# edsonportosilva/OptiCommPy

Hardware: AMD Instinct MI355X
Metric: SSFM steps/sec (2-pol, 2^20 samples) (higher is better)
Workload: dtype f64

## Files before the change

opticommpy_amd/csrc/engine_fused_impl.h:

```cpp
#pragma once
#include <algorithm>
#include <cstdlib>
#include <vector>

#include "dev_ctx.h"
#include "fused_engine.h"
#include "ssf_internal.h"

namespace ssf {
namespace {

using namespace fused;

#ifdef SSF_PHASE_TIMING
__device__ unsigned long long g_marks[4][4096][8];
#endif

struct DevCtx : DevCtxCore {
#ifdef SSF_PHASE_TIMING
    int kind;
    unsigned long long ts[8] = {0, 0, 0, 0, 0, 0, 0, 0};
    __device__ __forceinline__ void mark(int i) {
        __builtin_amdgcn_sched_barrier(0);
#if SSF_PHASE_TIMING != 2
// ... 689 lines not shown
        if (std::memcmp(k5, key, sizeof(key)) != 0) {
            const double w2 = (w_scale / (double)N) * (w_scale / (double)N);
            LinOp lo = make_linop(hzh, lin_a, lin_b, w2, scale, 4);
            be.h2d(lin_d, &lo, sizeof(LinOp));
            std::memcpy(key, k5, sizeof(key));
        }
        RowArgs<T> a{};
        a.G = (cx<T> *)out;
        a.src = in == out ? nullptr : (const cx<T> *)in;
        a.log2N1 = 0;
        a.log2N2 = 0;
        a.nfft = nrows;
        a.use_ctrl = 0;
        a.lin = lin_d;
        a.N2 = (int)N;
        a.N = N;
        a.mixed = 1;
        a.plan = plan;
        a.wtab = use_wtab ? wtab : nullptr;
        a.rows_per_wg = rows_wg;
        be.launch_row(a, nrows / rows_wg, tpr * rows_wg, 4096 + (size_t)rows_wg * (size_t)N * sizeof(cx<T>));
        return be.ok() ? SSF_OK : SSF_ERR_HIP;
    }
};

template <typename T>
int overlap_save_t(int64_t sigLen, int nrows, int lg, int K, const void *Hfft, const void *in, void *out, std::string *err) {
    using Cc = cx<T>;
    const int nfft = 1 << lg, d = nfft - K + 1, discard = K - 1, D = (K - 1) / 2;
    const long long numBlocks = (sigLen + K - 1 + d - 1) / d;
    const size_t sig_bytes = sizeof(Cc) * (size_t)sigLen * (size_t)nrows;
    hipStream_t st = nullptr;
    Cc *din = nullptr, *dout = nullptr, *dH = nullptr;
    auto fail_ = [&](const char *what, hipError_t e) {
        *err = std::string(what) + ": " + hipGetErrorString(e);
        if (din) (void)hipFree(din);
        if (dout) (void)hipFree(dout);
        if (dH) (void)hipFree(dH);
        if (st) (void)hipStreamDestroy(st);
        return e == hipErrorOutOfMemory ? SSF_ERR_OOM : SSF_ERR_HIP;
    };
    hipError_t e;
    if ((e = hipStreamCreateWithFlags(&st, hipStreamNonBlocking)) != hipSuccess) return fail_("hipStreamCreate", e);
    if ((e = hipMalloc(&din, sig_bytes)) != hipSuccess) return fail_("hipMalloc", e);
    if ((e = hipMalloc(&dout, sig_bytes)) != hipSuccess) return fail_("hipMalloc", e);
    if ((e = hipMalloc(&dH, sizeof(Cc) * (size_t)nfft)) != hipSuccess) return fail_("hipMalloc", e);
    std::vector<Cc> Hs((size_t)nfft);
    for (int i = 0; i < nfft; ++i) {
        Hs[(size_t)i].re = ((const Cc *)Hfft)[i].re / (T)nfft;
        Hs[(size_t)i].im = ((const Cc *)Hfft)[i].im / (T)nfft;
    }
    ols_permute_filter(Hs.data(), lg);
    Stager stg;
    (void)stg.init();
    if ((e = stg.h2d(din, in, sig_bytes, st)) != hipSuccess) return fail_("upload", e);
    if ((e = hipMemcpyAsync(dH, Hs.data(), sizeof(Cc) * (size_t)nfft, hipMemcpyHostToDevice, st)) != hipSuccess) return fail_("upload H", e);
    OlsArgs<T> a{};
    a.in = din;
    a.out = dout;
    a.H = dH;
    a.sigLen = sigLen;
    a.njobs = numBlocks * nrows;
    a.nrows = nrows;
    a.log2nfft = lg;
    a.d = d;
    a.discard = discard;
    a.D = D;
    ols_defaults(a);
    const int tpf = nfft / 16;
    const int block = tpf >= 256 ? tpf : 256, fpw = block / tpf;
    const long long grid = (a.njobs + fpw - 1) / fpw;
    const size_t lds = (size_t)fpw * lds_slots_per_fft(nfft) * sizeof(Cc);
    if (block <= 256) {
        (void)hipFuncSetAttribute((const void *)k_ols<T, 256>, hipFuncAttributeMaxDynamicSharedMemorySize, 160 * 1024);
        k_ols<T, 256><<<(unsigned)grid, block, lds, st>>>(a);
    } else {
        (void)hipFuncSetAttribute((const void *)k_ols<T, 1024>, hipFuncAttributeMaxDynamicSharedMemorySize, 160 * 1024);
        k_ols<T, 1024><<<(unsigned)grid, block, lds, st>>>(a);
    }
    if ((e = hipGetLastError()) != hipSuccess) return fail_("launch k_ols", e);
    if ((e = stg.d2h(out, dout, sig_bytes, st)) != hipSuccess) return fail_("download", e);
    (void)hipFree(din);
    (void)hipFree(dout);
    (void)hipFree(dH);
    (void)hipStreamDestroy(st);
    return SSF_OK;
}

inline int couple_reduce_selftest_impl(int nranks, int npart, const double *parts, double *out5, std::string *err) {
    if (nranks < 1 || npart < 1 || !parts || !out5) return SSF_ERR_BAD_ARG;
    double *d = nullptr, *work = nullptr;
    const size_t n = (size_t)nranks * 5 * (size_t)npart;
    hipError_t e = hipMalloc(&d, sizeof(double) * n);
    if (e == hipSuccess) e = hipMalloc(&work, sizeof(double) * (size_t)(8 + 5 * nranks));
    if (e == hipSuccess) e = hipMemcpy(d, parts, sizeof(double) * n, hipMemcpyHostToDevice);
    for (int r = 0; r < nranks && e == hipSuccess; ++r) {
        const double *b = d + (size_t)r * 5 * npart;
        CoupleArgs a{b + 3 * (size_t)npart, b + 4 * (size_t)npart, b + (size_t)npart, b + 2 * (size_t)npart, b, npart, work + 8 + 5 * r};
        k_couple_local<<<1, 256>>>(a);
        e = hipGetLastError();
    }
    if (e == hipSuccess) {
        k_couple_finish<<<1, 64>>>(work + 8, nranks, work);
        e = hipGetLastError();
    }
    if (e == hipSuccess) e = hipMemcpy(out5, work, sizeof(double) * 5, hipMemcpyDeviceToHost);
    if (d) (void)hipFree(d);
// ... 38 lines not shown
```

opticommpy_amd/csrc/engine_rx.hip:

```cpp
#include <cstring>
#include <set>
#include <string>
#include <utility>
#include <vector>

#include "dev_ctx.h"
#include "rx_pipeline.h"
#include "ssf_copy.h"
#include "ssf_internal.h"

namespace ssf {
namespace {

using namespace rx;

struct RxCtx : DevCtxCore {
    __device__ __forceinline__ void mark(int) {}
    __device__ __forceinline__ void flush(int) {}
};
#define SSF_RX_CTX()                                                          \
    extern __shared__ __attribute__((aligned(16))) char ssf_smem[];           \
    RxCtx ctx{{(int)threadIdx.x, (int)blockIdx.x, (int)blockDim.x, (int)gridDim.x, ssf_smem}}

template <int LG, int C> __global__ void __launch_bounds__(fused::ols_threads(LG, C)) k_rx_ols(const fused::OlsArgs<double> a) {
// ... 37 lines not shown
    absmax_body(ctx, a);
}
__global__ void __launch_bounds__(256) k_tx_phase_noise(const PnArgs a) {
    SSF_RX_CTX();
    pn_body(ctx, a);
}
__global__ void __launch_bounds__(256) k_tx_iqm(const IqmArgs a) {
    SSF_RX_CTX();
    iqm_body(ctx, a);
}
__global__ void __launch_bounds__(256) k_tx_shift_add(const ShiftAddArgs a) {
    SSF_RX_CTX();
    shift_add_body(ctx, a);
}
template <int LG, int C, int MODE> __global__ void __launch_bounds__(fused::ols_threads(LG, C)) k_rx_chain_ols(const ChainOlsArgs a) {
    SSF_RX_CTX();
    chain_ols_body<LG, C, MODE>(ctx, a);
}
__global__ void __launch_bounds__(1024) k_rx_chain_finish(const ChainFinishArgs a) {
    SSF_RX_CTX();
    chain_finish_body(ctx, a);
}
__global__ void __launch_bounds__(256) k_rx_dec_stats(const DecStatsArgs a) {
    SSF_RX_CTX();
    dec_stats_body(ctx, a);
}
__global__ void __launch_bounds__(256) k_rx_dec_sum(const DecSumArgs a) {
    SSF_RX_CTX();
    dec_sum_body(ctx, a);
}
__global__ void __launch_bounds__(256) k_rx_dec_finish(const DecFinishArgs a) {
    SSF_RX_CTX();
    dec_finish_body(ctx, a);
}
__global__ void __launch_bounds__(256) k_rx_dec_gather(const DecGatherArgs a) {
    SSF_RX_CTX();
    dec_gather_body(ctx, a);
}

struct HipRxBackend {
    hipStream_t st = nullptr;
    hipError_t first_err = hipSuccess;
    std::string where;
    Stager stg;
    void chk(hipError_t e, const char *what) {
        if (e != hipSuccess && first_err == hipSuccess) {
            first_err = e;
            where = what;
        }
    }
    int open(int device) {
        chk(hipSetDevice(device), "hipSetDevice");
        chk(hipStreamCreateWithFlags(&st, hipStreamNonBlocking), "hipStreamCreate");
        if (ok()) chk(stg.init(), "pinned staging buffers");
        return ok() ? SSF_OK : SSF_ERR_HIP;
    }
    ~HipRxBackend() {
        if (st) (void)hipStreamDestroy(st);
    }
    bool ok() const { return first_err == hipSuccess; }
    bool oom() const { return first_err == hipErrorOutOfMemory; }
    std::string last_error() const { return where + ": " + hipGetErrorString(first_err); }
    void *alloc(size_t n) {
        void *p = nullptr;
        hipError_t e = hipMalloc(&p, n);
        if (e != hipSuccess) {
            chk(e, "hipMalloc");
            return nullptr;
        }
        return p;
    }
    void free(void *p) { (void)hipFree(p); }
    void h2d(void *d, const void *h, size_t n) {
        chk(hipMemcpyAsync(d, h, n, hipMemcpyHostToDevice, st), "hipMemcpyAsync H2D");
        chk(hipStreamSynchronize(st), "hipStreamSynchronize");
    }
    void d2h(void *h, const void *d, size_t n) {
        chk(hipMemcpyAsync(h, d, n, hipMemcpyDeviceToHost, st), "hipMemcpyAsync D2H");
        chk(hipStreamSynchronize(st), "hipStreamSynchronize");
    }
    void h2d_big(void *d, const void *h, size_t n) { chk(stg.h2d(d, h, n, st), "staged upload"); }
    void d2h_big(void *h, const void *d, size_t n) { chk(stg.d2h(h, d, n, st), "staged download"); }
    void sync() { chk(hipStreamSynchronize(st), "hipStreamSynchronize"); }
    static unsigned ew_grid(long long n) {
        const long long g = (n + 255) / 256;
        return (unsigned)(g < 1 ? 1 : g > 4096 ? 4096 : g);
    }
    std::set<const void *> armed;
    template <class K> void arm(K kernel) {
        if (!armed.insert((const void *)kernel).second) return;
        chk(hipFuncSetAttribute((const void *)kernel, hipFuncAttributeMaxDynamicSharedMemorySize, 160 * 1024), "hipFuncSetAttribute");
    }
    void launch_ols(const fused::OlsArgs<double> &a) {
        const fused::OlsLaunch o = fused::ols_launch(a.log2nfft, a.nrows, a.njobs);
        fused::ols_dispatch(o, [&](auto lg, auto cc) {
            constexpr int LG = decltype(lg)::value, C = decltype(cc)::value;
            arm(k_rx_ols<LG, C>);
            k_rx_ols<LG, C><<<(unsigned)o.grid, o.threads, o.lds_bytes, st>>>(a);
        });
        chk(hipGetLastError(), "launch k_rx_ols");
    }
    void launch_rx_ols(const RxOlsArgs &a) {
        const fused::OlsLaunch o = fused::ols_launch(a.o.log2nfft, a.o.nrows, a.o.njobs);
        const bool found = rx_ols_dispatch(a, o, [&](auto lg, auto cc, auto pre, auto noise) {
            constexpr int LG = decltype(lg)::value, C = decltype(cc)::value, PRE = decltype(pre)::value, NOISE = decltype(noise)::value;
            arm(k_rx_ols_fused<LG, C, PRE, NOISE>);
            k_rx_ols_fused<LG, C, PRE, NOISE><<<(unsigned)o.grid, o.threads, o.lds_bytes, st>>>(a);
// ... 246 lines not shown
```

opticommpy_amd/csrc/ssf_api.hip:

```cpp
#include <map>
#include <memory>
#include <thread>

#include "ssf_internal.h"

using namespace ssf;

namespace {
thread_local std::string g_err;

int set_err(int code, const std::string &m) {
    g_err = m;
    return code;
}

int check_params(ssf_plan *pl, const ssf_params *p, int s0, int s1) {
    if (!p) return fail(pl, SSF_ERR_BAD_ARG, "params is NULL");
    if (p->model != SSF_MODEL_NLSE && p->model != SSF_MODEL_MANAKOV) return fail(pl, SSF_ERR_BAD_ARG, "bad model");
    if (p->model == SSF_MODEL_MANAKOV && (pl->nrows % 2)) return fail(pl, SSF_ERR_BAD_ARG, "Manakov model needs an even number of rows");
    if (p->model == SSF_MODEL_NLSE && p->direction < 0) return fail(pl, SSF_ERR_BAD_ARG, "NLSE model has no back-propagation mode");
    if (!(p->Fs > 0) || !(p->Fc > 0)) return fail(pl, SSF_ERR_BAD_ARG, "Fs and Fc must be positive");
    if (!(p->Lspan > 0)) return fail(pl, SSF_ERR_BAD_ARG, "Lspan must be positive");
    if (!(p->hz > 0) && !(p->model == SSF_MODEL_MANAKOV && p->nlprMethod)) return fail(pl, SSF_ERR_BAD_ARG, "hz must be positive");
    if (p->model == SSF_MODEL_MANAKOV && p->maxIter < 1) return fail(pl, SSF_ERR_BAD_ARG, "maxIter must be >= 1");
// ... 177 lines not shown
                ssf_stats *stats, ssf_trace *trace) {
    if (!plan) return set_err(SSF_ERR_BAD_ARG, "plan is NULL");
    if (!plan->has_field) return fail(plan, SSF_ERR_STATE, "ssf_execute before ssf_upload");
    int rc = check_params(plan, params, span_first, span_last);
    if (!rc && plan->sink.active()) {
        long long ncap = 0;
        for (int i = 0; i < params->n_save; ++i)
            if (params->save_spans[i] >= span_first && params->save_spans[i] <= span_last) ++ncap;
        if (((long long)plan->sink.count() + ncap) * plan->nrows > plan->sink.leading())
            return fail(plan, SSF_ERR_BAD_ARG, "snapshot sink: the captures of this call do not fit the destination's columns");
    }
    if (rc) return rc;
    SSF_HIP(plan, hipSetDevice(plan->device));
    if (trace) trace->count = 0;
    if (span_first <= span_last) {
        SSF_NEED_ENGINE(plan);
        rc = plan->engine->execute(*params, span_first, span_last, noise, &plan->stats, trace);
        if (rc) return rc;
    }
    const double s = plan->precision == SSF_C128 ? 16.0 : 8.0;
    plan->stats.bytes_algorithmic = (double)plan->stats.transforms * 2.0 * s * (double)plan->N;
    if (stats) *stats = plan->stats;
    return SSF_OK;
}

static int download_common(ssf_plan *plan, void *dst, int which, bool aos) {
    if (!plan) return set_err(SSF_ERR_BAD_ARG, "plan is NULL");
    if (!dst) return fail(plan, SSF_ERR_BAD_ARG, "destination is NULL");
    if (!plan->has_field) return fail(plan, SSF_ERR_STATE, "download before ssf_upload");
    SSF_NEED_ENGINE(plan);
    if (which < -1 || which >= plan->engine->n_snapshots()) return fail(plan, SSF_ERR_BAD_ARG, "no such snapshot");
    SSF_HIP(plan, hipSetDevice(plan->device));
    return plan->engine->download(dst, which, aos);
}
int ssf_download(ssf_plan *plan, void *field_soa) { return download_common(plan, field_soa, -1, false); }
int ssf_download_aos(ssf_plan *plan, int32_t which, void *field_aos) { return download_common(plan, field_aos, which, true); }

int ssf_download_snapshots(ssf_plan *plan, void *snap_soa) {
    if (!plan) return set_err(SSF_ERR_BAD_ARG, "plan is NULL");
    if (!snap_soa) return fail(plan, SSF_ERR_BAD_ARG, "snapshot buffer is NULL");
    const size_t fb = (size_t)plan->N * plan->nrows * (plan->precision == SSF_C128 ? 16 : 8);
    SSF_NEED_ENGINE(plan);
    for (int i = 0; i < plan->engine->n_snapshots(); ++i) {
        int rc = download_common(plan, (char *)snap_soa + (size_t)i * fb, i, false);
        if (rc) return rc;
    }
    return SSF_OK;
}

int ssf_set_snapshot_sink(ssf_plan *plan, void *dst, int64_t ld, int32_t first_index) {
    if (!plan) return set_err(SSF_ERR_BAD_ARG, "plan is NULL");
    if (dst && (ld < plan->nrows || first_index < 0)) return fail(plan, SSF_ERR_BAD_ARG, "ssf_set_snapshot_sink: ld < nrows or negative index");
    SSF_HIP(plan, hipSetDevice(plan->device));
    SSF_HIP(plan, plan->sink.set(plan->device, dst, ld, first_index, plan->precision == SSF_C128 ? 16 : 8));
    return SSF_OK;
}

int ssf_sync_snapshots(ssf_plan *plan) {
    if (!plan) return set_err(SSF_ERR_BAD_ARG, "plan is NULL");
    SSF_HIP(plan, hipSetDevice(plan->device));
    SSF_HIP(plan, hipStreamSynchronize(plan->stream));
    SSF_HIP(plan, plan->sink.sync());
    return SSF_OK;
}

int ssf_run(ssf_plan *plan, const ssf_params *params, const void *in, void *out, void *snaps, const void *noise,
            ssf_stats *stats, ssf_trace *trace) {
    int rc = ssf_upload(plan, in);
    if (rc) return rc;
    rc = ssf_execute(plan, params, 1, params ? params->Nspans : 0, noise, stats, trace);
    if (rc) return rc;
    if (out && (rc = ssf_download(plan, out))) return rc;
    if (snaps && plan->stats.n_snapshots > 0 && (rc = ssf_download_snapshots(plan, snaps))) return rc;
    return SSF_OK;
}

int ssf_set_coupling(ssf_plan *plan, ssf_reduce_fn reduce, void *ctx) {
    if (!plan) return set_err(SSF_ERR_BAD_ARG, "plan is NULL");
    SSF_NEED_ENGINE(plan);
    int rc = plan->engine->set_coupling(reduce, ctx);
    if (rc == SSF_OK) plan->coupled = reduce != nullptr;
    return rc ? fail(plan, rc, "coupled batches need the general-length engine (create the plan with SSF_ENGINE_ROCFFT)") : SSF_OK;
}

int ssf_set_coupling_comm(ssf_plan *plan, ssf_comm *comm) {
    if (!plan) return set_err(SSF_ERR_BAD_ARG, "plan is NULL");
    SSF_NEED_ENGINE(plan);
    if (comm && ssf::comm_device(comm) != plan->device) return fail(plan, SSF_ERR_BAD_ARG, "ssf_set_coupling_comm: the communicator lives on another device");
    if (comm && plan->units > 1) return fail(plan, SSF_ERR_UNSUPPORTED, "ssf_set_coupling_comm: a plan of independent units is not a coupled batch");
    int rc = plan->engine->set_coupling_comm(comm);
    if (rc == SSF_OK) plan->coupled = comm != nullptr;
    return rc ? fail(plan, rc, "device-side coupling needs the device-resident fused pipeline (else: ssf_set_coupling on SSF_ENGINE_ROCFFT)") : SSF_OK;
}

static int rx_check_device(int device);
int ssf_couple_reduce_selftest(int device, int32_t nranks, int32_t npart, const double *parts, double *out5) {
    if (int rc = rx_check_device(device)) return rc;
    if (hipSetDevice(device) != hipSuccess) return set_err(SSF_ERR_HIP, "hipSetDevice");
    std::string err;
    int rc = ssf::fused_couple_reduce_selftest(nranks, npart, parts, out5, &err);
    return rc ? set_err(rc, err.empty() ? "ssf_couple_reduce_selftest: bad argument" : err) : SSF_OK;
}

int ssf_set_profiling(ssf_plan *plan, int32_t enable) {
    if (!plan) return set_err(SSF_ERR_BAD_ARG, "plan is NULL");
    SSF_NEED_ENGINE(plan);
    int rc = plan->engine->set_profiling(enable);
// ... 149 lines not shown
                    rc = ssf_run(pl, &pu, (const char *)fields_in + (size_t)u * unit_bytes,
                                 (char *)fields_out + (size_t)u * unit_bytes, nullptr, nullptr, &st, nullptr);
                    if (stats) stats[u] = st;
                }
                if (rc) {
                    rcs[(size_t)slot] = rc;
                    errs[(size_t)slot] = ssf_last_error(pl);
                }
                ssf_plan_destroy(pl);
            });
        }
    }
    for (auto &t : th) t.join();
    for (int i = 0; i < nslots; ++i)
        if (rcs[(size_t)i]) return set_err(rcs[(size_t)i], "device " + std::to_string(dev_ids[i / lanes]) + ": " + errs[(size_t)i]);
    return SSF_OK;
}

int ssf_device_malloc(int device, int64_t bytes, void **ptr) {
    if (!ptr || bytes < 1) return set_err(SSF_ERR_BAD_ARG, "ssf_device_malloc: bad argument");
    int ndev = 0;
    if (hipGetDeviceCount(&ndev) != hipSuccess || device < 0 || device >= ndev) return set_err(SSF_ERR_NO_DEVICE, "device index out of range");
    if (hipSetDevice(device) != hipSuccess) return set_err(SSF_ERR_HIP, "hipSetDevice failed");
    hipError_t e = hipMalloc(ptr, (size_t)bytes);
    if (e != hipSuccess) return set_err(e == hipErrorOutOfMemory ? SSF_ERR_OOM : SSF_ERR_HIP, std::string("hipMalloc: ") + hipGetErrorString(e));
    return SSF_OK;
}

int ssf_device_free(int device, void *ptr) {
    if (!ptr) return SSF_OK;
    if (hipSetDevice(device) != hipSuccess) return set_err(SSF_ERR_HIP, "hipSetDevice failed");
    hipError_t e = hipFree(ptr);
    return e == hipSuccess ? SSF_OK : set_err(SSF_ERR_HIP, std::string("hipFree: ") + hipGetErrorString(e));
}

int ssf_device_memcpy(int device, void *dst, const void *src, int64_t bytes) {
    if (!dst || !src || bytes < 0) return set_err(SSF_ERR_BAD_ARG, "ssf_device_memcpy: bad argument");
    if (hipSetDevice(device) != hipSuccess) return set_err(SSF_ERR_HIP, "hipSetDevice failed");
    const bool dst_dev = ssf::on_device(dst), src_dev = ssf::on_device(src);
    hipError_t e;
    if (dst_dev != src_dev && bytes >= (1 << 20)) {
        struct Lane {
            hipStream_t st = nullptr;
            ssf::Stager stg;
        };
        thread_local std::map<int, std::unique_ptr<Lane>> lanes;
        std::unique_ptr<Lane> &slot = lanes[device];
        if (!slot) {
            slot.reset(new Lane());
            if (hipStreamCreateWithFlags(&slot->st, hipStreamNonBlocking) != hipSuccess) {
                slot.reset();
                return set_err(SSF_ERR_HIP, "hipStreamCreate failed");
            }
            (void)slot->stg.init();
        }
        Lane &lane = *slot;
        e = dst_dev ? lane.stg.h2d(dst, src, (size_t)bytes, lane.st) : lane.stg.d2h(dst, src, (size_t)bytes, lane.st);
    } else {
        e = hipMemcpy(dst, src, (size_t)bytes, hipMemcpyDefault);
    }
    return e == hipSuccess ? SSF_OK : set_err(SSF_ERR_HIP, std::string("ssf_device_memcpy: ") + hipGetErrorString(e));
}

static int rx_check_device(int device) {
    int ndev = 0;
    if (hipGetDeviceCount(&ndev) != hipSuccess || ndev == 0) return set_err(SSF_ERR_NO_DEVICE, "no HIP device visible");
    if (device < 0 || device >= ndev) return set_err(SSF_ERR_NO_DEVICE, "device index out of range");
    return SSF_OK;
}

int ssf_fir_filter(int device, int64_t sigLen, int32_t ncols, int32_t ntaps, const void *taps, const void *in, void *out) {
    if (!taps || !in || !out) return set_err(SSF_ERR_BAD_ARG, "ssf_fir_filter: NULL argument");
    if (int rc = rx_check_device(device)) return rc;
    std::string err;
    int rc = ssf::rx_fir(device, sigLen, ncols, ntaps, taps, in, out, &err);
    return rc ? set_err(rc, "ssf_fir_filter: " + err) : SSF_OK;
}

int ssf_fir_long(int device, int64_t inLen, int64_t outLen, int32_t ncols, int64_t ntaps, const void *taps, int64_t shift,
                 const void *in, void *out) {
    if (!taps || !in || !out) return set_err(SSF_ERR_BAD_ARG, "ssf_fir_long: NULL argument");
    if (int rc = rx_check_device(device)) return rc;
    std::string err;
    int rc = ssf::rx_fir_long(device, inLen, outLen, ncols, ntaps, taps, shift, in, out, &err);
    return rc ? set_err(rc, "ssf_fir_long: " + err) : SSF_OK;
}

int ssf_device_axpy(int device, int64_t n, double alpha, const double *x, double *y) {
    if (!x || !y) return set_err(SSF_ERR_BAD_ARG, "ssf_device_axpy: NULL argument");
    if (int rc = rx_check_device(device)) return rc;
    std::string err;
    int rc = ssf::rx_axpy(device, n, alpha, x, y, &err);
    return rc ? set_err(rc, "ssf_device_axpy: " + err) : SSF_OK;
}

int ssf_delay_signal(int device, int64_t N, double delay, double Fs, const void *in, void *out) {
    if (!in || !out) return set_err(SSF_ERR_BAD_ARG, "ssf_delay_signal: NULL argument");
    if (int rc = rx_check_device(device)) return rc;
    std::string err;
    int rc = ssf::rx_delay(device, N, delay, Fs, in, out, &err);
    return rc ? set_err(rc, "ssf_delay_signal: " + err) : SSF_OK;
}

int ssf_edfa(int device, int64_t n, int32_t ncols, double G_lin, double p_noise, int64_t rng_seed, int32_t rng_row_offset,
             const void *field_in, const void *noise, void *field_out) {
    if (!field_in || !field_out || n < 1 || ncols < 1) return set_err(SSF_ERR_BAD_ARG, "ssf_edfa: bad argument");
    if (!(G_lin > 0) || p_noise < 0) return set_err(SSF_ERR_BAD_ARG, "ssf_edfa: the gain must be positive, the noise power non-negative");
// ... 217 lines not shown
```

opticommpy_amd/csrc/ssf_copy.h:

```cpp
#pragma once
#include <hip/hip_runtime.h>

#include <cstring>

namespace ssf {

template <typename C> __global__ void k_aos_to_soa(const C *aos, C *soa, long long N, int nrows) {
    const long long total = N * nrows;
    for (long long i = blockIdx.x * (long long)blockDim.x + threadIdx.x; i < total; i += (long long)gridDim.x * blockDim.x) {
        const long long n = i / nrows;
        const int r = (int)(i - n * nrows);
        soa[(long long)r * N + n] = aos[i];
    }
}
template <typename C> __global__ void k_soa_to_aos(const C *soa, C *aos, long long N, int nrows) {
    const long long total = N * nrows;
    for (long long i = blockIdx.x * (long long)blockDim.x + threadIdx.x; i < total; i += (long long)gridDim.x * blockDim.x) {
        const long long n = i / nrows;
        const int r = (int)(i - n * nrows);
        aos[i] = soa[(long long)r * N + n];
    }
}

inline bool on_device(const void *p) {
    hipPointerAttribute_t a;
    if (hipPointerGetAttributes(&a, p) != hipSuccess) {
        (void)hipGetLastError();
        return false;
    }
    return a.type == hipMemoryTypeDevice;
}

class Stager {
    static constexpr size_t kChunk = 8u << 20;
    void *pin[2] = {nullptr, nullptr};
    hipEvent_t ev[2] = {nullptr, nullptr};
    bool ok_ = false;

  public:
    hipError_t init() {
        for (int i = 0; i < 2; ++i) {
            hipError_t e = hipHostMalloc(&pin[i], kChunk);
            if (e != hipSuccess) return e;
            e = hipEventCreateWithFlags(&ev[i], hipEventDisableTiming);
            if (e != hipSuccess) return e;
        }
        ok_ = true;
        return hipSuccess;
    }
    ~Stager() {
        for (int i = 0; i < 2; ++i) {
            if (pin[i]) (void)hipHostFree(pin[i]);
            if (ev[i]) (void)hipEventDestroy(ev[i]);
        }
    }
    hipError_t h2d(void *dev, const void *host, size_t n, hipStream_t s) {
        if (on_device(host)) {
            hipError_t e = hipMemcpyAsync(dev, host, n, hipMemcpyDeviceToDevice, s);
            return e != hipSuccess ? e : hipStreamSynchronize(s);
        }
        if (!ok_ || n < (1u << 20)) {
            hipError_t e = hipMemcpyAsync(dev, host, n, hipMemcpyHostToDevice, s);
            return e != hipSuccess ? e : hipStreamSynchronize(s);
        }
        size_t off = 0;
        for (int i = 0; off < n; ++i, off += kChunk) {
            const int b = i & 1;
            const size_t len = n - off < kChunk ? n - off : kChunk;
            if (i >= 2) {
                hipError_t e = hipEventSynchronize(ev[b]);
                if (e != hipSuccess) return e;
            }
            std::memcpy(pin[b], (const char *)host + off, len);
            hipError_t e = hipMemcpyAsync((char *)dev + off, pin[b], len, hipMemcpyHostToDevice, s);
            if (e != hipSuccess) return e;
            if ((e = hipEventRecord(ev[b], s)) != hipSuccess) return e;
        }
        return hipStreamSynchronize(s);
    }
    hipError_t d2h(void *host, const void *dev, size_t n, hipStream_t s) {
        if (on_device(host)) {
            hipError_t e = hipMemcpyAsync(host, dev, n, hipMemcpyDeviceToDevice, s);
            return e != hipSuccess ? e : hipStreamSynchronize(s);
        }
        if (!ok_ || n < (1u << 20)) {
            hipError_t e = hipMemcpyAsync(host, dev, n, hipMemcpyDeviceToHost, s);
            return e != hipSuccess ? e : hipStreamSynchronize(s);
        }
        const int nchunks = (int)((n + kChunk - 1) / kChunk);
        for (int i = 0; i <= nchunks; ++i) {
            if (i < nchunks) {
                const int b = i & 1;
                const size_t off = (size_t)i * kChunk, len = n - off < kChunk ? n - off : kChunk;
                hipError_t e = hipMemcpyAsync(pin[b], (const char *)dev + off, len, hipMemcpyDeviceToHost, s);
                if (e != hipSuccess) return e;
                if ((e = hipEventRecord(ev[b], s)) != hipSuccess) return e;
            }
            if (i >= 1) {
                const int b = (i - 1) & 1;
                const size_t off = (size_t)(i - 1) * kChunk, len = n - off < kChunk ? n - off : kChunk;
                hipError_t e = hipEventSynchronize(ev[b]);
                if (e != hipSuccess) return e;
                std::memcpy((char *)host + off, pin[b], len);
            }
        }
        return hipSuccess;
    }
};

}
```

opticommpy_amd/csrc/ssf_snapshots.h:

```cpp
#pragma once
#include <hip/hip_runtime.h>

#include <algorithm>
#include <condition_variable>
#include <cstring>
#include <deque>
#include <mutex>
#include <string>
#include <thread>

#include "ssf_copy.h"

namespace ssf {

template <typename C> __global__ void k_soa_to_cols(const C *soa, C *out, long long N, int nrows, long long ld, long long col0) {
    const long long total = N * nrows;
    for (long long i = blockIdx.x * (long long)blockDim.x + threadIdx.x; i < total; i += (long long)gridDim.x * blockDim.x) {
        const long long n = i / nrows;
        const int r = (int)(i - n * nrows);
        out[n * ld + col0 + r] = soa[(long long)r * N + n];
    }
}

class SnapshotSink {
    static constexpr size_t kChunk = 8u << 20;
    struct Job {
        int buf;
        long long N, col0;
        int nrows;
    };
    int device = 0;
    char *dst = nullptr;
    long long ld = 0;
    size_t esz = 16;
    bool dst_dev = false;
    int index = 0;
    void *stage[2] = {nullptr, nullptr};
    size_t stage_cap[2] = {0, 0};
    hipEvent_t ready[2] = {nullptr, nullptr};
    bool busy[2] = {false, false};
    void *pin[2] = {nullptr, nullptr};
    hipEvent_t pin_ev[2] = {nullptr, nullptr};
    hipStream_t copy_st = nullptr;
    std::thread worker;
    std::mutex mu;
    std::condition_variable cv;
    std::deque<Job> jobs;
    int inflight = 0;
    bool stop = false, started = false;
    hipError_t first_err = hipSuccess;

    void note(hipError_t e) {
        if (e != hipSuccess && first_err == hipSuccess) first_err = e;
    }
    void run() {
        (void)hipSetDevice(device);
        for (;;) {
            Job j;
            {
                std::unique_lock<std::mutex> lk(mu);
                cv.wait(lk, [&] { return stop || !jobs.empty(); });
                if (jobs.empty()) return;
                j = jobs.front();
                jobs.pop_front();
            }
            hipError_t e = hipEventSynchronize(ready[j.buf]);
            const size_t row = (size_t)j.nrows * esz;
            const long long rows_per_chunk = std::max<long long>(1, (long long)(kChunk / row));
            const long long nchunks = (j.N + rows_per_chunk - 1) / rows_per_chunk;
            for (long long i = 0; e == hipSuccess && i <= nchunks; ++i) {
                if (i < nchunks) {
                    const int b = (int)(i & 1);
                    const long long r0 = i * rows_per_chunk, nr = std::min(rows_per_chunk, j.N - r0);
                    e = hipMemcpyAsync(pin[b], (const char *)stage[j.buf] + (size_t)r0 * row, (size_t)nr * row, hipMemcpyDeviceToHost, copy_st);
                    if (e == hipSuccess) e = hipEventRecord(pin_ev[b], copy_st);
                }
                if (e == hipSuccess && i >= 1) {
                    const int b = (int)((i - 1) & 1);
                    const long long r0 = (i - 1) * rows_per_chunk, nr = std::min(rows_per_chunk, j.N - r0);
                    e = hipEventSynchronize(pin_ev[b]);
                    if (e == hipSuccess) {
                        const char *src = (const char *)pin[b];
                        char *d = dst + ((size_t)r0 * (size_t)ld + (size_t)j.col0) * esz;
                        if ((long long)j.nrows == ld) std::memcpy(d, src, (size_t)nr * row);
                        else
                            for (long long r = 0; r < nr; ++r) std::memcpy(d + (size_t)r * (size_t)ld * esz, src + (size_t)r * row, row);
                    }
                }
            }
            {
                std::lock_guard<std::mutex> lk(mu);
                note(e);
                busy[j.buf] = false;
                --inflight;
            }
            cv.notify_all();
        }
    }
    hipError_t start() {
        if (started) return hipSuccess;
        hipError_t e = copy_st ? hipSuccess : hipStreamCreateWithFlags(&copy_st, hipStreamNonBlocking);
        for (int i = 0; i < 2 && e == hipSuccess; ++i) {
            if (!pin[i]) e = hipHostMalloc(&pin[i], kChunk);
            if (e == hipSuccess && !pin_ev[i]) e = hipEventCreateWithFlags(&pin_ev[i], hipEventDisableTiming);
            if (e == hipSuccess && !ready[i]) e = hipEventCreateWithFlags(&ready[i], hipEventDisableTiming);
        }
        if (e != hipSuccess) return e;
        worker = std::thread([this] { run(); });
        started = true;
        return hipSuccess;
    }

  public:
    SnapshotSink() = default;
    SnapshotSink(const SnapshotSink &) = delete;
    ~SnapshotSink() {
        (void)sync();
        if (started) {
            {
                std::lock_guard<std::mutex> lk(mu);
                stop = true;
            }
            cv.notify_all();
            worker.join();
        }
        for (int i = 0; i < 2; ++i) {
            if (stage[i]) (void)hipFree(stage[i]);
            if (pin[i]) (void)hipHostFree(pin[i]);
            if (pin_ev[i]) (void)hipEventDestroy(pin_ev[i]);
            if (ready[i]) (void)hipEventDestroy(ready[i]);
        }
        if (copy_st) (void)hipStreamDestroy(copy_st);
    }
    bool active() const { return dst != nullptr; }
    int count() const { return index; }
    long long leading() const { return ld; }
    hipError_t set(int dev, void *d, long long ld_, int first_index, size_t elem_size) {
        hipError_t e = sync();
        device = dev;
        dst = (char *)d;
        ld = ld_;
        index = first_index;
        esz = elem_size;
        dst_dev = d && on_device(d);
        return e;
    }
    template <typename C> hipError_t capture(const C *soa, long long N, int nrows, hipStream_t st) {
        if (((long long)index + 1) * nrows > ld || (size_t)nrows * esz > kChunk) return hipErrorInvalidValue;
        const long long col0 = (long long)index * nrows;
        ++index;
        if (dst_dev) {
            k_soa_to_cols<C><<<1024, 256, 0, st>>>(soa, (C *)dst, N, nrows, ld, col0);
            return hipGetLastError();
        }
        hipError_t e = start();
        if (e != hipSuccess) return e;
        int b;
        {
            std::unique_lock<std::mutex> lk(mu);
            cv.wait(lk, [&] { return !busy[0] || !busy[1]; });
            b = !busy[0] ? 0 : 1;
            busy[b] = true;
            ++inflight;
        }
        const size_t bytes = (size_t)N * (size_t)nrows * sizeof(C);
        if (stage_cap[b] < bytes) {
            if (stage[b]) (void)hipFree(stage[b]);
            stage[b] = nullptr;
            stage_cap[b] = 0;
            if ((e = hipMalloc(&stage[b], bytes)) == hipSuccess) stage_cap[b] = bytes;
        }
        if (e == hipSuccess) {
            k_soa_to_cols<C><<<1024, 256, 0, st>>>(soa, (C *)stage[b], N, nrows, (long long)nrows, 0);
            e = hipGetLastError();
        }
        if (e == hipSuccess) e = hipEventRecord(ready[b], st);
        {
            std::lock_guard<std::mutex> lk(mu);
            if (e == hipSuccess) jobs.push_back(Job{b, N, col0, nrows});
            else {
                busy[b] = false;
                --inflight;
            }
        }
        cv.notify_all();
        return e;
    }
    hipError_t sync() {
        if (!started) return hipSuccess;
        std::unique_lock<std::mutex> lk(mu);
        cv.wait(lk, [&] { return inflight == 0; });
        const hipError_t e = first_err;
        first_err = hipSuccess;
        return e;
    }
};

}
```

Baseline: 6324.

## Parallelize host staging copies with a thread pool and deeper pinned ring

Replaces the two-buffer pinned staging with a configurable-depth pinned ring and a small host thread pool that splits the memcpy into and out of pinned memory across several threads. Pinned buffer allocation is deferred until the first large transfer, and the snapshot sink prefaults the host destination with MADV_POPULATE_WRITE in the background. The aim is to cut host-side memcpy and page-fault costs in upload, download and snapshot paths. It adds threads, more pinned memory and synchronisation complexity. None of this touches the per-step GPU kernels, so steps/sec is likely unaffected unless the timing includes transfers.

```diff
diff --git a/opticommpy_amd/csrc/engine_fused_impl.h b/opticommpy_amd/csrc/engine_fused_impl.h
--- a/opticommpy_amd/csrc/engine_fused_impl.h
+++ b/opticommpy_amd/csrc/engine_fused_impl.h
@@ -765,7 +765,7 @@
     }
     ols_permute_filter(Hs.data(), lg);
     Stager stg;
-    (void)stg.init();
+    stg.defer();
     if ((e = stg.h2d(din, in, sig_bytes, st)) != hipSuccess) return fail_("upload", e);
     if ((e = hipMemcpyAsync(dH, Hs.data(), sizeof(Cc) * (size_t)nfft, hipMemcpyHostToDevice, st)) != hipSuccess) return fail_("upload H", e);
     OlsArgs<T> a{};
diff --git a/opticommpy_amd/csrc/engine_rx.hip b/opticommpy_amd/csrc/engine_rx.hip
--- a/opticommpy_amd/csrc/engine_rx.hip
+++ b/opticommpy_amd/csrc/engine_rx.hip
@@ -113,7 +113,7 @@
     int open(int device) {
         chk(hipSetDevice(device), "hipSetDevice");
         chk(hipStreamCreateWithFlags(&st, hipStreamNonBlocking), "hipStreamCreate");
-        if (ok()) chk(stg.init(), "pinned staging buffers");
+        stg.defer();
         return ok() ? SSF_OK : SSF_ERR_HIP;
     }
     ~HipRxBackend() {
diff --git a/opticommpy_amd/csrc/host_copy_pool.h b/opticommpy_amd/csrc/host_copy_pool.h
--- /dev/null
+++ b/opticommpy_amd/csrc/host_copy_pool.h
@@ -0,0 +1,183 @@
+#pragma once
+#include <sys/mman.h>
+
+#include <condition_variable>
+#include <cstddef>
+#include <cstdint>
+#include <cstring>
+#include <mutex>
+#include <thread>
+#include <vector>
+
+namespace ssf {
+namespace hostcopy {
+
+constexpr size_t kPage = 4096;
+constexpr int kMaxWorkers = 4;
+constexpr size_t kMinSlice = 64 * kPage;
+
+struct Slice {
+    size_t off, len;
+};
+
+inline int split(size_t len, int parts, Slice *out) {
+    if (len == 0) return 0;
+    if (parts < 1) parts = 1;
+    const size_t pages = (len + kPage - 1) / kPage;
+    size_t per = ((pages + (size_t)parts - 1) / (size_t)parts) * kPage;
+    if (per < kMinSlice) per = kMinSlice;
+    int n = 0;
+    for (size_t off = 0; off < len; off += per) out[n++] = Slice{off, len - off < per ? len - off : per};
+    return n;
+}
+
+inline size_t chunk_bytes(size_t chunk, size_t row) {
+    if (row == 0 || row >= chunk) return row ? row : chunk;
+    return chunk / row * row;
+}
+inline size_t chunk_count(size_t n, size_t chunk) { return (n + chunk - 1) / chunk; }
+inline Slice chunk_at(size_t n, size_t chunk, size_t i) {
+    const size_t off = i * chunk;
+    return Slice{off, n - off < chunk ? n - off : chunk};
+}
+
+#ifndef MADV_POPULATE_WRITE
+#define MADV_POPULATE_WRITE 23
+#endif
+inline void populate_write(void *p, size_t len) {
+    const uintptr_t a = ((uintptr_t)p + kPage - 1) & ~(uintptr_t)(kPage - 1), b = ((uintptr_t)p + len) & ~(uintptr_t)(kPage - 1);
+    if (b > a) (void)madvise((void *)a, (size_t)(b - a), MADV_POPULATE_WRITE);
+}
+
+class CopyPool {
+    std::vector<std::thread> th;
+    std::mutex mu, run_mu;
+    std::condition_variable cv_work, cv_done;
+    void (*fn)(void *, int) = nullptr;
+    void *ctx = nullptr;
+    int nparts = 0, next = 0, pending = 0;
+    bool stop = false;
+
+    void worker() {
+        std::unique_lock<std::mutex> lk(mu);
+        for (;;) {
+            cv_work.wait(lk, [&] { return stop || next < nparts; });
+            if (stop) return;
+            take(lk);
+        }
+    }
+    void take(std::unique_lock<std::mutex> &lk) {
+        const int p = next++;
+        void (*f)(void *, int) = fn;
+        void *c = ctx;
+        lk.unlock();
+        f(c, p);
+        lk.lock();
+        if (--pending == 0) cv_done.notify_all();
+    }
+
+  public:
+    explicit CopyPool(int workers = kMaxWorkers) {
+        if (workers > kMaxWorkers) workers = kMaxWorkers;
+        for (int i = 1; i < workers; ++i) th.emplace_back([this] { worker(); });
+    }
+    CopyPool(const CopyPool &) = delete;
+    CopyPool &operator=(const CopyPool &) = delete;
+    ~CopyPool() {
+        {
+            std::lock_guard<std::mutex> lk(mu);
+            stop = true;
+        }
+        cv_work.notify_all();
+        for (auto &t : th) t.join();
+    }
+    int workers() const { return (int)th.size() + 1; }
+
+    void run(int parts, void (*f)(void *, int), void *c) {
+        if (parts <= 0) return;
+        if (parts == 1 || th.empty()) {
+            for (int p = 0; p < parts; ++p) f(c, p);
+            return;
+        }
+        std::lock_guard<std::mutex> one(run_mu);
+        std::unique_lock<std::mutex> lk(mu);
+        fn = f;
+        ctx = c;
+        nparts = pending = parts;
+        next = 0;
+        cv_work.notify_all();
+        while (next < nparts) take(lk);
+        cv_done.wait(lk, [&] { return pending == 0; });
+        nparts = next = 0;
+    }
+
+    void copy(void *dst, const void *src, size_t len) {
+        struct Job {
+            char *d;
+            const char *s;
+            Slice sl[kMaxWorkers];
+        } j{(char *)dst, (const char *)src, {}};
+        const int n = split(len, workers(), j.sl);
+        run(n, [](void *c, int p) {
+            Job *q = (Job *)c;
+            std::memcpy(q->d + q->sl[p].off, q->s + q->sl[p].off, q->sl[p].len);
+        }, &j);
+    }
+    void populate(void *dst, size_t len) {
+        struct Job {
+            char *d;
+            Slice sl[kMaxWorkers];
+        } j{(char *)dst, {}};
+        const int n = split(len, workers(), j.sl);
+        run(n, [](void *c, int p) {
+            Job *q = (Job *)c;
+            populate_write(q->d + q->sl[p].off, q->sl[p].len);
+        }, &j);
+    }
+    void scatter_rows(void *dst, size_t stride, const void *src, size_t row, size_t rows) {
+        if (stride == row) return copy(dst, src, row * rows);
+        struct Job {
+            char *d;
+            const char *s;
+            size_t stride, row, rows, per;
+        } j{(char *)dst, (const char *)src, stride, row, rows, 0};
+        int n = workers();
+        if (rows * row < 2 * kMinSlice) n = 1;
+        j.per = (rows + (size_t)n - 1) / (size_t)n;
+        n = j.per ? (int)((rows + j.per - 1) / j.per) : 0;
+        run(n, [](void *c, int p) {
+            Job *q = (Job *)c;
+            const size_t r0 = (size_t)p * q->per, r1 = r0 + q->per < q->rows ? r0 + q->per : q->rows;
+            for (size_t r = r0; r < r1; ++r) std::memcpy(q->d + r * q->stride, q->s + r * q->row, q->row);
+        }, &j);
+    }
+};
+
+template <class Wait, class Fill, class Send> int ring_upload(size_t nchunks, int depth, Wait wait, Fill fill, Send send) {
+    for (size_t i = 0; i < nchunks; ++i) {
+        const int b = (int)(i % (size_t)depth);
+        if (i >= (size_t)depth)
+            if (int e = wait(b)) return e;
+        fill(b, i);
+        if (int e = send(b, i)) return e;
+    }
+    return 0;
+}
+template <class Fetch, class Wait, class Drain> int ring_download(size_t nchunks, int depth, Fetch fetch, Wait wait, Drain drain) {
+    size_t fetched = 0;
+    for (; fetched < nchunks && fetched < (size_t)depth; ++fetched)
+        if (int e = fetch((int)fetched, fetched)) return e;
+    for (size_t i = 0; i < nchunks; ++i) {
+        const int b = (int)(i % (size_t)depth);
+        if (int e = wait(b)) return e;
+        drain(b, i);
+        if (fetched < nchunks) {
+            if (int e = fetch(b, fetched)) return e;
+            ++fetched;
+        }
+    }
+    return 0;
+}
+
+}
+}
diff --git a/opticommpy_amd/csrc/ssf_api.hip b/opticommpy_amd/csrc/ssf_api.hip
--- a/opticommpy_amd/csrc/ssf_api.hip
+++ b/opticommpy_amd/csrc/ssf_api.hip
@@ -253,7 +253,7 @@
     if (!plan) return set_err(SSF_ERR_BAD_ARG, "plan is NULL");
     if (dst && (ld < plan->nrows || first_index < 0)) return fail(plan, SSF_ERR_BAD_ARG, "ssf_set_snapshot_sink: ld < nrows or negative index");
     SSF_HIP(plan, hipSetDevice(plan->device));
-    SSF_HIP(plan, plan->sink.set(plan->device, dst, ld, first_index, plan->precision == SSF_C128 ? 16 : 8));
+    SSF_HIP(plan, plan->sink.set(plan->device, dst, ld, first_index, plan->precision == SSF_C128 ? 16 : 8, plan->N));
     return SSF_OK;
 }
 
@@ -509,7 +509,7 @@
                 slot.reset();
                 return set_err(SSF_ERR_HIP, "hipStreamCreate failed");
             }
-            (void)slot->stg.init();
+            (void)slot->stg.init(4u << 20);
         }
         Lane &lane = *slot;
         e = dst_dev ? lane.stg.h2d(dst, src, (size_t)bytes, lane.st) : lane.stg.d2h(dst, src, (size_t)bytes, lane.st);
diff --git a/opticommpy_amd/csrc/ssf_copy.h b/opticommpy_amd/csrc/ssf_copy.h
--- a/opticommpy_amd/csrc/ssf_copy.h
+++ b/opticommpy_amd/csrc/ssf_copy.h
@@ -2,6 +2,9 @@
 #include <hip/hip_runtime.h>
 
 #include <cstring>
+#include <memory>
+
+#include "host_copy_pool.h"
 
 namespace ssf {
 
@@ -31,80 +34,115 @@
     return a.type == hipMemoryTypeDevice;
 }
 
-class Stager {
-    static constexpr size_t kChunk = 8u << 20;
-    void *pin[2] = {nullptr, nullptr};
-    hipEvent_t ev[2] = {nullptr, nullptr};
-    bool ok_ = false;
+struct PinnedRing {
+    static constexpr int kMaxDepth = 8;
+    size_t chunk = 0;
+    int depth = 0;
+    void *pin[kMaxDepth] = {};
+    hipEvent_t ev[kMaxDepth] = {};
 
-  public:
-    hipError_t init() {
-        for (int i = 0; i < 2; ++i) {
-            hipError_t e = hipHostMalloc(&pin[i], kChunk);
+    hipError_t init(size_t chunk_bytes, int n) {
+        if (depth) return hipSuccess;
+        if (n < 2 || n > kMaxDepth || chunk_bytes < hostcopy::kPage) return hipErrorInvalidValue;
+        for (int i = 0; i < n; ++i) {
+            hipError_t e = pin[i] ? hipSuccess : hipHostMalloc(&pin[i], chunk_bytes);
+            if (e == hipSuccess && !ev[i]) e = hipEventCreateWithFlags(&ev[i], hipEventDisableTiming);
             if (e != hipSuccess) return e;
-            e = hipEventCreateWithFlags(&ev[i], hipEventDisableTiming);
-            if (e != hipSuccess) return e;
+            std::memset(pin[i], 0, chunk_bytes);
         }
-        ok_ = true;
+        chunk = chunk_bytes;
+        depth = n;
         return hipSuccess;
     }
-    ~Stager() {
-        for (int i = 0; i < 2; ++i) {
+    ~PinnedRing() {
+        for (int i = 0; i < kMaxDepth; ++i) {
             if (pin[i]) (void)hipHostFree(pin[i]);
             if (ev[i]) (void)hipEventDestroy(ev[i]);
         }
+    }
+    PinnedRing() = default;
+    PinnedRing(const PinnedRing &) = delete;
+    PinnedRing &operator=(const PinnedRing &) = delete;
+};
+
+class Stager {
+  public:
+    static constexpr size_t kChunk = 8u << 20;
+    static constexpr int kDepth = 4;
+
+  private:
+    PinnedRing ring;
+    std::unique_ptr<hostcopy::CopyPool> pool;
+    bool ok_ = false, deferred_ = false;
+
+  public:
+    void defer() { deferred_ = true; }
+    hipError_t init(size_t chunk = kChunk, int depth = kDepth, int workers = hostcopy::kMaxWorkers) {
+        if (ok_) return hipSuccess;
+        hipError_t e = ring.init(chunk, depth);
+        if (e != hipSuccess) return e;
+        pool.reset(new hostcopy::CopyPool(workers));
+        ok_ = true;
+        return hipSuccess;
     }
     hipError_t h2d(void *dev, const void *host, size_t n, hipStream_t s) {
         if (on_device(host)) {
             hipError_t e = hipMemcpyAsync(dev, host, n, hipMemcpyDeviceToDevice, s);
             return e != hipSuccess ? e : hipStreamSynchronize(s);
         }
+        if (deferred_ && n >= (1u << 20)) {
+            deferred_ = false;
+            (void)init();
+        }
         if (!ok_ || n < (1u << 20)) {
             hipError_t e = hipMemcpyAsync(dev, host, n, hipMemcpyHostToDevice, s);
             return e != hipSuccess ? e : hipStreamSynchronize(s);
         }
-        size_t off = 0;
-        for (int i = 0; off < n; ++i, off += kChunk) {
-            const int b = i & 1;
-            const size_t len = n - off < kChunk ? n - off : kChunk;
-            if (i >= 2) {
-                hipError_t e = hipEventSynchronize(ev[b]);
-                if (e != hipSuccess) return e;
-            }
-            std::memcpy(pin[b], (const char *)host + off, len);
-            hipError_t e = hipMemcpyAsync((char *)dev + off, pin[b], len, hipMemcpyHostToDevice, s);
-            if (e != hipSuccess) return e;
-            if ((e = hipEventRecord(ev[b], s)) != hipSuccess) return e;
-        }
-        return hipStreamSynchronize(s);
+        const size_t chunk = ring.chunk;
+        const int rc = hostcopy::ring_upload(
+            hostcopy::chunk_count(n, chunk), ring.depth, [&](int b) { return (int)hipEventSynchronize(ring.ev[b]); },
+            [&](int b, size_t i) {
+                const hostcopy::Slice c = hostcopy::chunk_at(n, chunk, i);
+                pool->copy(ring.pin[b], (const char *)host + c.off, c.len);
+            },
+            [&](int b, size_t i) {
+                const hostcopy::Slice c = hostcopy::chunk_at(n, chunk, i);
+                hipError_t e = hipMemcpyAsync((char *)dev + c.off, ring.pin[b], c.len, hipMemcpyHostToDevice, s);
+                if (e == hipSuccess) e = hipEventRecord(ring.ev[b], s);
+                return (int)e;
+            });
+        const hipError_t e = hipStreamSynchronize(s);
+        return rc ? (hipError_t)rc : e;
     }
     hipError_t d2h(void *host, const void *dev, size_t n, hipStream_t s) {
         if (on_device(host)) {
             hipError_t e = hipMemcpyAsync(host, dev, n, hipMemcpyDeviceToDevice, s);
             return e != hipSuccess ? e : hipStreamSynchronize(s);
         }
+        if (deferred_ && n >= (1u << 20)) {
+            deferred_ = false;
+            (void)init();
+        }
         if (!ok_ || n < (1u << 20)) {
             hipError_t e = hipMemcpyAsync(host, dev, n, hipMemcpyDeviceToHost, s);
             return e != hipSuccess ? e : hipStreamSynchronize(s);
         }
-        const int nchunks = (int)((n + kChunk - 1) / kChunk);
-        for (int i = 0; i <= nchunks; ++i) {
-            if (i < nchunks) {
-                const int b = i & 1;
-                const size_t off = (size_t)i * kChunk, len = n - off < kChunk ? n - off : kChunk;
-                hipError_t e = hipMemcpyAsync(pin[b], (const char *)dev + off, len, hipMemcpyDeviceToHost, s);
-                if (e != hipSuccess) return e;
-                if ((e = hipEventRecord(ev[b], s)) != hipSuccess) return e;
-            }
-            if (i >= 1) {
-                const int b = (i - 1) & 1;
-                const size_t off = (size_t)(i - 1) * kChunk, len = n - off < kChunk ? n - off : kChunk;
-                hipError_t e = hipEventSynchronize(ev[b]);
-                if (e != hipSuccess) return e;
-                std::memcpy((char *)host + off, pin[b], len);
-            }
-        }
-        return hipSuccess;
+        const size_t chunk = ring.chunk;
+        const int rc = hostcopy::ring_download(
+            hostcopy::chunk_count(n, chunk), ring.depth,
+            [&](int b, size_t i) {
+                const hostcopy::Slice c = hostcopy::chunk_at(n, chunk, i);
+                hipError_t e = hipMemcpyAsync(ring.pin[b], (const char *)dev + c.off, c.len, hipMemcpyDeviceToHost, s);
+                if (e == hipSuccess) e = hipEventRecord(ring.ev[b], s);
+                return (int)e;
+            },
+            [&](int b) { return (int)hipEventSynchronize(ring.ev[b]); },
+            [&](int b, size_t i) {
+                const hostcopy::Slice c = hostcopy::chunk_at(n, chunk, i);
+                pool->copy((char *)host + c.off, ring.pin[b], c.len);
+            });
+        if (rc) (void)hipStreamSynchronize(s);
+        return (hipError_t)rc;
     }
 };
 
diff --git a/opticommpy_amd/csrc/ssf_snapshots.h b/opticommpy_amd/csrc/ssf_snapshots.h
--- a/opticommpy_amd/csrc/ssf_snapshots.h
+++ b/opticommpy_amd/csrc/ssf_snapshots.h
@@ -5,6 +5,7 @@
 #include <condition_variable>
 #include <cstring>
 #include <deque>
+#include <memory>
 #include <mutex>
 #include <string>
 #include <thread>
@@ -23,11 +24,12 @@
 }
 
 class SnapshotSink {
-    static constexpr size_t kChunk = 8u << 20;
+    static constexpr size_t kChunk = Stager::kChunk;
     struct Job {
         int buf;
         long long N, col0;
         int nrows;
+        size_t prefault;
     };
     int device = 0;
     char *dst = nullptr;
@@ -39,8 +41,8 @@
     size_t stage_cap[2] = {0, 0};
     hipEvent_t ready[2] = {nullptr, nullptr};
     bool busy[2] = {false, false};
-    void *pin[2] = {nullptr, nullptr};
-    hipEvent_t pin_ev[2] = {nullptr, nullptr};
+    PinnedRing ring;
+    std::unique_ptr<hostcopy::CopyPool> pool;
     hipStream_t copy_st = nullptr;
     std::thread worker;
     std::mutex mu;
@@ -64,29 +66,33 @@
                 j = jobs.front();
                 jobs.pop_front();
             }
+            if (j.prefault) {
+                pool->populate(dst, j.prefault);
+                std::lock_guard<std::mutex> lk(mu);
+                --inflight;
+                cv.notify_all();
+                continue;
+            }
             hipError_t e = hipEventSynchronize(ready[j.buf]);
             const size_t row = (size_t)j.nrows * esz;
-            const long long rows_per_chunk = std::max<long long>(1, (long long)(kChunk / row));
-            const long long nchunks = (j.N + rows_per_chunk - 1) / rows_per_chunk;
-            for (long long i = 0; e == hipSuccess && i <= nchunks; ++i) {
-                if (i < nchunks) {
-                    const int b = (int)(i & 1);
-                    const long long r0 = i * rows_per_chunk, nr = std::min(rows_per_chunk, j.N - r0);
-                    e = hipMemcpyAsync(pin[b], (const char *)stage[j.buf] + (size_t)r0 * row, (size_t)nr * row, hipMemcpyDeviceToHost, copy_st);
-                    if (e == hipSuccess) e = hipEventRecord(pin_ev[b], copy_st);
-                }
-                if (e == hipSuccess && i >= 1) {
-                    const int b = (int)((i - 1) & 1);
-                    const long long r0 = (i - 1) * rows_per_chunk, nr = std::min(rows_per_chunk, j.N - r0);
-                    e = hipEventSynchronize(pin_ev[b]);
-                    if (e == hipSuccess) {
-                        const char *src = (const char *)pin[b];
-                        char *d = dst + ((size_t)r0 * (size_t)ld + (size_t)j.col0) * esz;
-                        if ((long long)j.nrows == ld) std::memcpy(d, src, (size_t)nr * row);
-                        else
-                            for (long long r = 0; r < nr; ++r) std::memcpy(d + (size_t)r * (size_t)ld * esz, src + (size_t)r * row, row);
-                    }
-                }
+            const size_t chunk = hostcopy::chunk_bytes(kChunk, row), total = (size_t)j.N * row;
+            if (e == hipSuccess) {
+                const int rc = hostcopy::ring_download(
+                    hostcopy::chunk_count(total, chunk), ring.depth,
+                    [&](int b, size_t i) {
+                        const hostcopy::Slice c = hostcopy::chunk_at(total, chunk, i);
+                        hipError_t q = hipMemcpyAsync(ring.pin[b], (const char *)stage[j.buf] + c.off, c.len, hipMemcpyDeviceToHost, copy_st);
+                        if (q == hipSuccess) q = hipEventRecord(ring.ev[b], copy_st);
+                        return (int)q;
+                    },
+                    [&](int b) { return (int)hipEventSynchronize(ring.ev[b]); },
+                    [&](int b, size_t i) {
+                        const hostcopy::Slice c = hostcopy::chunk_at(total, chunk, i);
+                        char *d = dst + ((size_t)(c.off / row) * (size_t)ld + (size_t)j.col0) * esz;
+                        pool->scatter_rows(d, (size_t)ld * esz, ring.pin[b], row, c.len / row);
+                    });
+                e = (hipError_t)rc;
+                if (rc) (void)hipStreamSynchronize(copy_st);
             }
             {
                 std::lock_guard<std::mutex> lk(mu);
@@ -100,12 +106,11 @@
     hipError_t start() {
         if (started) return hipSuccess;
         hipError_t e = copy_st ? hipSuccess : hipStreamCreateWithFlags(&copy_st, hipStreamNonBlocking);
-        for (int i = 0; i < 2 && e == hipSuccess; ++i) {
-            if (!pin[i]) e = hipHostMalloc(&pin[i], kChunk);
-            if (e == hipSuccess && !pin_ev[i]) e = hipEventCreateWithFlags(&pin_ev[i], hipEventDisableTiming);
-            if (e == hipSuccess && !ready[i]) e = hipEventCreateWithFlags(&ready[i], hipEventDisableTiming);
-        }
+        if (e == hipSuccess) e = ring.init(kChunk, Stager::kDepth);
+        for (int i = 0; i < 2 && e == hipSuccess; ++i)
+            if (!ready[i]) e = hipEventCreateWithFlags(&ready[i], hipEventDisableTiming);
         if (e != hipSuccess) return e;
+        if (!pool) pool.reset(new hostcopy::CopyPool());
         worker = std::thread([this] { run(); });
         started = true;
         return hipSuccess;
@@ -126,8 +131,6 @@
         }
         for (int i = 0; i < 2; ++i) {
             if (stage[i]) (void)hipFree(stage[i]);
-            if (pin[i]) (void)hipHostFree(pin[i]);
-            if (pin_ev[i]) (void)hipEventDestroy(pin_ev[i]);
             if (ready[i]) (void)hipEventDestroy(ready[i]);
         }
         if (copy_st) (void)hipStreamDestroy(copy_st);
@@ -135,7 +138,7 @@
     bool active() const { return dst != nullptr; }
     int count() const { return index; }
     long long leading() const { return ld; }
-    hipError_t set(int dev, void *d, long long ld_, int first_index, size_t elem_size) {
+    hipError_t set(int dev, void *d, long long ld_, int first_index, size_t elem_size, long long N = 0) {
         hipError_t e = sync();
         device = dev;
         dst = (char *)d;
@@ -143,6 +146,14 @@
         index = first_index;
         esz = elem_size;
         dst_dev = d && on_device(d);
+        if (d && !dst_dev && N > 0 && start() == hipSuccess) {
+            {
+                std::lock_guard<std::mutex> lk(mu);
+                ++inflight;
+                jobs.push_back(Job{0, N, 0, 0, (size_t)N * (size_t)ld * esz});
+            }
+            cv.notify_all();
+        }
         return e;
     }
     template <typename C> hipError_t capture(const C *soa, long long N, int nrows, hipStream_t st) {
@@ -177,7 +188,7 @@
         if (e == hipSuccess) e = hipEventRecord(ready[b], st);
         {
             std::lock_guard<std::mutex> lk(mu);
-            if (e == hipSuccess) jobs.push_back(Job{b, N, col0, nrows});
+            if (e == hipSuccess) jobs.push_back(Job{b, N, col0, nrows, 0});
             else {
                 busy[b] = false;
                 --inflight;
```

New measurement: 6330, median of 4. Within noise of the previous version (+0.1%).
